# liuzl/rwkv-tts-rs

Measured on AMD Instinct MI355X. Metric: audio samples/sec (16 kHz) for RWKV-TTS 0.4B, batch=32 per GPU, higher is better.
Workload: dtype bf16; 1 GPU; config3: 32 requests/GPU, P=32 prompt, 32 global + 512 semantic tokens, exact sampler, + BiCodec vocoder -> PCM (vocoder of batch s overlapped with LM of batch s+1 on its own stream); global_batch=32, seq_len=577, parallelism=dp1 (request sharding)

## Files before the change

### rwkv-tts-rs_amd/csrc/sampler.hip

```cpp
#include "sampler.h"
#include "exact_math.h"

namespace rwkvtts {

__device__ inline uint32_t rotl32(uint32_t x, int n) { return (x << n) | (x >> (32 - n)); }
#define QR(a, b, c, d)               \
  a += b; d ^= a; d = rotl32(d, 16); \
  c += d; b ^= c; b = rotl32(b, 12); \
  a += b; d ^= a; d = rotl32(d, 8);  \
  c += d; b ^= c; b = rotl32(b, 7);

__device__ uint32_t chacha12_word(const uint32_t* key, uint64_t index) {
  uint32_t in[16] = {0x61707865u, 0x3320646eu, 0x79622d32u, 0x6b206574u};
  for (int i = 0; i < 8; ++i) in[4 + i] = key[i];
  const uint64_t ctr = index >> 4;
  in[12] = (uint32_t)ctr;
  in[13] = (uint32_t)(ctr >> 32);
  in[14] = 0;
  in[15] = 0;
  uint32_t x[16];
  for (int i = 0; i < 16; ++i) x[i] = in[i];
  for (int i = 0; i < 12; i += 2) {
    QR(x[0], x[4], x[8], x[12]);
    QR(x[1], x[5], x[9], x[13]);
// ... 163 lines not shown
}
__device__ inline float prefix64(float s, float v, float* total) {
  float out = 0.0f;
  const int lane = threadIdx.x & 63;
#pragma unroll 8
  for (int i = 0; i < 64; ++i) {
    s += readlane_f(v, i);
    out = lane == i ? s : out;
  }
  *total = s;
  return out;
}

struct SampleSmem {
  float* p;
  uint64_t* keys;
  int* list;
  int* scan;
  double* dscan;
  uint32_t* sub_t;
  int* sub_e;
  int* chunk_e;
  uint32_t* chunk_t;
  int* chunk_ok;
  int* runs;
  uint64_t* etab;
  float* fred;
  int* ired;
  int cap;
};

__device__ inline int wave_sum_i(int v) {
  for (int o = 32; o >= 1; o >>= 1) v += __shfl_xor(v, o);
  return v;
}

template <int NT>
__device__ inline float block_max(float v, float* fred) {
  for (int o = 32; o >= 1; o >>= 1) v = fmaxf(v, __shfl_xor(v, o));
  __syncthreads();
  if ((threadIdx.x & 63) == 0) fred[threadIdx.x >> 6] = v;
  __syncthreads();
  float m = fred[0];
#pragma unroll
  for (int w = 1; w < NT / 64; ++w) m = fmaxf(m, fred[w]);
  return m;
}

template <int N>
__device__ inline int dpp_shr(int v) {
  return __builtin_amdgcn_update_dpp(0, v, 0x110 + N, 0xF, 0xF, false);
}
template <int N>
__device__ inline double dpp_shr(double v) {
  const uint64_t u = __builtin_bit_cast(uint64_t, v);
  const uint32_t lo = (uint32_t)dpp_shr<N>((int)(uint32_t)u), hi = (uint32_t)dpp_shr<N>((int)(uint32_t)(u >> 32));
  return __builtin_bit_cast(double, ((uint64_t)hi << 32) | lo);
}
template <int N>
__device__ inline uint32_t dpp_shr(uint32_t v) {
  return (uint32_t)dpp_shr<N>((int)v);
}
__device__ inline double readlane_d(double v, int l) {
  const uint64_t u = __builtin_bit_cast(uint64_t, v);
  const uint32_t lo = (uint32_t)__builtin_amdgcn_readlane((int)(uint32_t)u, l);
  const uint32_t hi = (uint32_t)__builtin_amdgcn_readlane((int)(uint32_t)(u >> 32), l);
  return __builtin_bit_cast(double, ((uint64_t)hi << 32) | lo);
}
__device__ inline double wave_incl_scan_d(double x) {
  x += dpp_shr<1>(x);
  x += dpp_shr<2>(x);
  x += dpp_shr<4>(x);
  x += dpp_shr<8>(x);
  const double r0 = readlane_d(x, 15), r1 = readlane_d(x, 31), r2 = readlane_d(x, 47);
  const int row = (threadIdx.x & 63) >> 4;
  return x + (row == 0 ? 0.0 : (row == 1 ? r0 : (row == 2 ? r0 + r1 : (r0 + r1) + r2)));
}

__device__ inline uint64_t readlane_u64(uint64_t v, int l) {
  const uint32_t lo = (uint32_t)__builtin_amdgcn_readlane((int)(uint32_t)v, l);
  const uint32_t hi = (uint32_t)__builtin_amdgcn_readlane((int)(uint32_t)(v >> 32), l);
  return ((uint64_t)hi << 32) | lo;
}
template <typename KeyAt>
__device__ inline int wave_rank_gt(uint64_t q, int m, const KeyAt& key_at) {
  const int lane = threadIdx.x & 63;
  int rank = 0;
  for (int j0 = 0; j0 < m; j0 += 64) {
    const uint64_t kl = j0 + lane < m ? key_at(j0 + lane) : 0ull;
#pragma unroll
    for (int j = 0; j < 64; ++j) rank += readlane_u64(kl, j) > q ? 1 : 0;
  }
  return rank;
}
__device__ inline int readlane_t(int v, int l) { return __builtin_amdgcn_readlane(v, l); }
__device__ inline uint32_t readlane_t(uint32_t v, int l) { return (uint32_t)__builtin_amdgcn_readlane((int)v, l); }
__device__ inline double readlane_t(double v, int l) { return readlane_d(v, l); }

template <int NT, typename T>
__device__ inline T block_excl_scan_t(T v, T* scratch, T* tot) {
  const int lane = threadIdx.x & 63, w = threadIdx.x >> 6;
  T x = v;
  x += dpp_shr<1>(x);
  x += dpp_shr<2>(x);
  x += dpp_shr<4>(x);
  x += dpp_shr<8>(x);
  {
    const T r0 = readlane_t(x, 15), r1 = readlane_t(x, 31), r2 = readlane_t(x, 47);
    const int row = lane >> 4;
    const T off = row == 0 ? (T)0 : (row == 1 ? r0 : (row == 2 ? r0 + r1 : (r0 + r1) + r2));
    x += off;
  }
  __syncthreads();
  if (lane == 63) scratch[w] = x;
  __syncthreads();
  T base = 0;
  for (int k = 0; k < w; ++k) base += scratch[k];
  T t = scratch[0];
#pragma unroll
  for (int k = 1; k < NT / 64; ++k) t += scratch[k];
  *tot = t;
  return base + x - v;
}
template <int NT>
__device__ inline int block_excl_scan(int v, int* scratch, int* tot) { return block_excl_scan_t<NT, int>(v, scratch, tot); }

template <int NT>
__device__ int compact_positive_(const float* p, int* list, int* scan, int cap, int n) {
  const int chunk = (n + NT - 1) / NT;
  const int b = min(n, (int)threadIdx.x * chunk), e = min(n, b + chunk);
  int cnt = 0;
  for (int i = b; i < e; ++i) cnt += p[i] > 0.0f;
  int tot;
  int off = block_excl_scan<NT>(cnt, scan, &tot);
  for (int i = b; i < e; ++i)
    if (p[i] > 0.0f) {
      if (off < cap) list[off] = i;
      ++off;
    }
  __syncthreads();
  return tot;
}
template <int NT>
__device__ inline int compact_positive(const SampleSmem& sm, int n) {
  return compact_positive_<NT>(sm.p, sm.list, sm.scan, sm.cap, n);
}

__device__ float wave_sum_positive_(const float* p, const int* list, int cap, int n, int npos) {
  const int lane = threadIdx.x & 63;
  float s = 0.0f;
  if (npos <= cap) {
    for (int q0 = 0; q0 < npos; q0 += 64) {
      const float v = (q0 + lane < npos) ? p[list[q0 + lane]] : 0.0f;
      const int cnt = min(64, npos - q0);
      for (int i = 0; i < cnt; ++i) s += readlane_f(v, i);
    }
  } else {
    for (int q0 = 0; q0 < n; q0 += 64) {
      const float v = (q0 + lane < n) ? p[q0 + lane] : 0.0f;
      const int cnt = min(64, n - q0);
      for (int i = 0; i < cnt; ++i) s += readlane_f(v, i);
    }
  }
  return s;
}
__device__ inline float wave_sum_positive(const SampleSmem& sm, int n, int npos) {
  return wave_sum_positive_(sm.p, sm.list, sm.cap, n, npos);
}

__device__ inline void sum_sim_elem(uint32_t b, int E, uint32_t& T0, uint32_t& T1, int& q0, int& q1, bool& ok) {
  const uint32_t ef = (b >> 23) & 0xFFu;
  uint32_t M = b & 0x7FFFFFu;
  int ex;
  if (ef == 0) ex = -149;
  else { M |= 0x800000u; ex = (int)ef - 150; }
  uint32_t a = 0;
  int cls = 0;
  if (M != 0) {
    const int sh = (E - 23) - ex;
    if (sh <= 0) {
// ... 319 lines not shown
      const uint32_t T1 = (uint32_t)readlane_i((int)(hiw ? b1 : b0), l);
      if (rs < pos) {
        serial(pos, re);
        pos = max(pos, re);
        continue;
      }
      serial(pos, rs);
      s = __builtin_bit_cast(float, __builtin_amdgcn_readfirstlane(__builtin_bit_cast(int, s)));
      const uint32_t sb = __builtin_bit_cast(uint32_t, s);
      const int ef = (int)((sb >> 23) & 0xFFu);
      const uint32_t mm = (sb & 0x7FFFFFu) | 0x800000u;
      const uint32_t T = (mm & 1u) ? T1 : T0;
      if (ef != 0 && ef - 127 == k + kRunEMin && mm + T < 0x1000000u)
        s = __builtin_bit_cast(float, (sb & 0xFF800000u) | ((mm + T) & 0x7FFFFFu));
      else
        serial(rs, re);
      pos = re;
    }
    serial(pos, n);
    if (tid == 0) {
      sm.fred[16] = s;
      if (stamps) {
        stamps[14] = __builtin_amdgcn_s_memtime();
        stamps[15] = sadd;
      }
    }
  } else {
    other();
  }
  __syncthreads();
  STAMP(13);
  return sm.fred[16];
}

template <int NT, typename Other = NoOther>
__device__ __attribute__((always_inline)) float exact_seq_sum(const SampleSmem& sm, int n, uint64_t* stamps = nullptr, const Other& other = Other()) {
  if (n <= kSampleMaxN) return exact_seq_sum_runs<NT>(sm, n, stamps, other);
  return exact_seq_sum_chunks<NT>(sm, n, stamps, other);
}

template <int NT>
__device__ void bitonic_desc(uint64_t* keys, int M) {
  for (int k = 2; k <= M; k <<= 1) {
    for (int j = k >> 1; j > 0; j >>= 1) {
      for (int q = threadIdx.x; q < M; q += NT) {
        const int ixj = q ^ j;
        if (ixj > q) {
          const uint64_t A = keys[q], B = keys[ixj];
          const bool desc = (q & k) == 0;
          if (desc ? (A < B) : (A > B)) { keys[q] = B; keys[ixj] = A; }
        }
      }
      __syncthreads();
    }
  }
}

template <int NT>
__device__ void sort_desc_u32(uint32_t* v, int n) {
  int M = 1;
  while (M < n) M <<= 1;
  for (int k = 2; k <= M; k <<= 1) {
    for (int j = k >> 1; j > 0; j >>= 1) {
      const bool flip = j == (k >> 1);
      for (int t = threadIdx.x; t < (M >> 1); t += NT) {
        const int q = ((t & ~(j - 1)) << 1) | (t & (j - 1));
        const int ixj = flip ? (q ^ (2 * j - 1)) : (q | j);
        if (ixj < n) {
          const uint32_t A = v[q], B = v[ixj];
          if (A < B) { v[q] = B; v[ixj] = A; }
        }
      }
      __syncthreads();
    }
  }
}

__device__ inline uint64_t pkey(float p, int i) {
  return ((uint64_t)__builtin_bit_cast(uint32_t, p) << 32) | (uint64_t)(0xFFFFFFFFu - (uint32_t)i);
}

constexpr int kSampleMaxVals = (kSampleMaxSorted * 8 + 16 * 8 + kSampleMaxSorted * 4) / 4;
constexpr int kFastK = kFastTopK;
constexpr int kFastCap = 1024;
static_assert(kSampleMaxSorted >= 2048 + kFastCap, "fast-path key regions");

__device__ inline bool sample_fast_ok(float sum, float L, int nc, int top_k) {
  if (!(sum > 0.0f) || !(L > 0.0f) || nc < top_k || nc > kFastCap) return false;
  const float P = L / sum;
  return P >= 0x1p-126f && P <= 1.0f;
}

__device__ inline float draw_r(const uint32_t* key, uint64_t draw, bool fixed42) {
  if (!fixed42) return draw_f32(key, draw);
  uint32_t k42[8];
  uint64_t st = 42;
  const uint64_t MUL = 6364136223846793005ull, INC = 11634580456473284103ull;
  for (int i = 0; i < 8; ++i) {
    st = st * MUL + INC;
    const uint32_t xs = (uint32_t)(((st >> 18) ^ st) >> 27);
    const uint32_t rot = (uint32_t)(st >> 59);
    k42[i] = (xs >> rot) | (xs << ((32 - rot) & 31));
  }
  return draw_f32(k42, 0);
}

template <int NT>
__device__ __attribute__((always_inline)) int sample_fast(const SampleSmem& sm, int nc, float sum, float top_p,
                                                          int top_k, float tinv, const uint32_t* key, uint64_t draw,
                                                          bool fixed42, float* dbg, uint64_t* stamps) {
  const int tid = threadIdx.x;
  uint64_t* pk = sm.keys + 2048;
  for (int c = tid; c < nc; c += NT) {
    const uint64_t ce = sm.keys[c];
    pk[c] = pkey(__builtin_bit_cast(float, (uint32_t)(ce >> 32)) / sum, (int)(uint32_t)ce);
  }
  __syncthreads();
  STAMP(4);
  for (int c = tid; c < nc; c += NT) {
    const uint64_t kc = pk[c];
    int rank = 0;
    for (int j = 0; j < nc; ++j) rank += pk[j] > kc ? 1 : 0;
    if (rank < top_k) sm.keys[rank] = kc;
  }
  __syncthreads();
  STAMP(5);
  STAMP(6);
  if (tid < 64) {
    int m = top_k, found = 0, ceq = 0;
    float cutoff = 0.0f;
    if (top_p < 1.0f) {
      float cum = 0.0f;
      for (int q0 = 0; q0 < top_k && !found; q0 += 64) {
        const bool in = q0 + tid < top_k;
        const float pv = in ? __builtin_bit_cast(float, (uint32_t)(sm.keys[q0 + tid] >> 32)) : 0.0f;
        float tot;
        const float pre = prefix64(cum, pv, &tot);
        const uint64_t hit = __ballot(in && pre >= top_p);
        if (hit) {
          found = 1;
          cutoff = readlane_f(pv, __builtin_ctzll(hit));
        }
        cum = tot;
      }
      if (found) {
        m = 0;
        for (int q0 = 0; q0 < top_k; q0 += 64) {
          const bool in = q0 + tid < top_k;
          const float pv = in ? __builtin_bit_cast(float, (uint32_t)(sm.keys[q0 + tid] >> 32)) : 0.0f;
          m += __popcll(__ballot(in && pv >= cutoff));
          ceq += __popcll(__ballot(in && pv == cutoff));
        }
      }
    }
    if (tid == 0) {
      sm.ired[2] = found;
      sm.ired[3] = ceq;
      sm.ired[6] = m;
      sm.fred[17] = cutoff;
    }
  }
  __syncthreads();
  const int m = sm.ired[6];
  for (int t = tid; t < m; t += NT) {
    const uint64_t kt = sm.keys[t];
    const uint32_t lt = (uint32_t)kt;
// ... 71 lines not shown
        for (int q0 = 0; q0 < m && ret < 0; q0 += 64) {
          const bool in = q0 + tid < m;
          const int idx_l = in ? sm.list[q0 + tid] : 0;
          const float v = in ? sm.p[idx_l] : 0.0f;
          float tot;
          const float pre = prefix64(cum, v, &tot);
          const uint64_t hit = __ballot(in && r <= pre);
          const uint64_t posm = __ballot(in && v > 0.0f);
          if (posm) last_pos = readlane_i(idx_l, 63 - __builtin_clzll(posm));
          if (hit) ret = readlane_i(idx_l, __builtin_ctzll(hit));
          cum = tot;
        }
        if (ret < 0) ret = max(last_pos, 0);
      }
      if (tid == 0) {
        sm.ired[5] = ret;
        if (dbg) { dbg[0] = sum; dbg[1] = r; }
      }
    }
    __syncthreads();
    STAMP(9);
    return sm.ired[5];
  }
  if (tid < 64) {
    const int found = sm.ired[2], ceq = sm.ired[3];
    const float cutoff = sm.fred[17];
    bool adj_on = false;
    float adj = 0.0f;
    if (top_p < 1.0f && found && top_p > 0.0f) {
      float s2 = 0.0f;
      for (int q0 = 0; q0 < m; q0 += 64) {
        const float v = q0 + tid < m ? sm.p[sm.list[q0 + tid]] : 0.0f;
        const int cnt = min(64, m - q0);
        for (int i = 0; i < cnt; ++i) s2 += readlane_f(v, i);
      }
      if (s2 < top_p && ceq > 0) {
        adj = (top_p - s2) / (float)ceq;
        adj_on = true;
      }
    }
    const float r = sm.fred[21];
    int ret = -1;
    if (r <= 0.0f) {
      ret = 0;
    } else {
      float cum = 0.0f;
      for (int q0 = 0; q0 < m && ret < 0; q0 += 64) {
        const bool in = q0 + tid < m;
        const int idx_l = in ? sm.list[q0 + tid] : 0;
        float v = in ? sm.p[idx_l] : 0.0f;
        if (adj_on && in && v == cutoff) v = cutoff + adj;
        float tot;
        const float pre = prefix64(cum, v, &tot);
        const uint64_t hit = __ballot(in && r <= pre);
        if (hit) ret = readlane_i(idx_l, __builtin_ctzll(hit));
        cum = tot;
      }
      if (ret < 0) ret = sm.list[m - 1];
    }
    if (tid == 0) {
      sm.ired[5] = ret;
      if (dbg) { dbg[0] = sum; dbg[1] = r; }
    }
  }
  __syncthreads();
  STAMP(9);
  return sm.ired[5];
}

__device__ inline double crude_sum_eps(int n) { return (double)n * 0x1p-23 + 0x1p-36; }

template <int NT>
__device__ __attribute__((always_inline)) int sample_cert(const SampleSmem& sm, int n, int nc, double E, float r, float top_p, int top_k,
                           double eps, uint64_t* stamps = nullptr) {
  const int tid = threadIdx.x;
  STAMP(7);
  uint64_t* srt = sm.keys + 2048;
  uint64_t* idx_o = sm.keys + 3072;
  static_assert(kSampleMaxSorted >= 3072 + kFastK, "certified-path key regions");
  auto qkey = [&](int j) {
    const uint64_t kj = sm.keys[j];
    return (kj & 0xFFFFFFFF00000000ull) | (uint64_t)(0xFFFFFFFFu - (uint32_t)kj);
  };
  for (int c0 = 0; c0 < nc; c0 += NT) {
    if (c0 + (tid & ~63) >= nc) break;
    const int c = c0 + tid;
    const uint64_t qc = c < nc ? qkey(c) : ~0ull;
    const int rank = wave_rank_gt(qc, nc, qkey);
    if (c < nc) srt[rank] = qc;
  }
  __syncthreads();
  STAMP(8);
  for (int t0 = 0; t0 < top_k; t0 += NT) {
    if (t0 + (tid & ~63) >= top_k) break;
    const int t = t0 + tid;
    const uint64_t kt = t < top_k ? srt[t] : 0ull;
    const uint32_t it = 0xFFFFFFFFu - (uint32_t)kt;
    auto nkey = [&](int j) { return (uint64_t)(uint32_t)srt[j]; };
    const int ri = wave_rank_gt((uint64_t)(uint32_t)kt, top_k, nkey);
    if (t < top_k) idx_o[ri] = (kt & 0xFFFFFFFF00000000ull) | it;
  }
  __syncthreads();
  STAMP(9);
  int ret = -1;
  if (tid < 64) {
    const double s_lo = E * (1.0 - eps), s_hi = E * (1.0 + eps);
    const double u = 0x1p-24, ua = 0x1p-23;
    bool ok = E > 0.0 && s_lo > 0.0 && E < 3.0e38;
    const float ek = __builtin_bit_cast(float, (uint32_t)(srt[top_k - 1] >> 32));
    if (ok && nc > top_k) {
      const float eb = __builtin_bit_cast(float, (uint32_t)(srt[top_k] >> 32));
      ok = (double)ek >= (double)eb * (1.0 + 0x1p-22);
    }
    ok = ok && (double)ek / s_hi >= 0x1p-120;
    double tot_hi = 0.0;
    for (int q0 = 0; q0 < top_k; q0 += 64) {
      const double e = q0 + tid < top_k ? (double)__builtin_bit_cast(float, (uint32_t)(idx_o[q0 + tid] >> 32)) : 0.0;
      tot_hi += readlane_d(wave_incl_scan_d(e), 63);
    }
    tot_hi = tot_hi / s_lo * (1.0 + u) * (1.0 + (double)top_k * ua);
    if (top_p < 1.0f) ok = ok && tot_hi < (double)top_p;
    STAMP(12);
    if (ok) {
      if (r <= 0.0f) {
        ret = 0;
      } else {
        double plo = 0.0, phi = 0.0, hi_prev = 0.0;
        bool amb = false;
        for (int q0 = 0; q0 < top_k && ret < 0 && !amb; q0 += 64) {
          const bool in = q0 + tid < top_k;
          const uint64_t kv = in ? idx_o[q0 + tid] : 0ull;
          const double e = in ? (double)__builtin_bit_cast(float, (uint32_t)(kv >> 32)) : 0.0;
          const double a = wave_incl_scan_d(e / s_hi * (1.0 - u)), b = wave_incl_scan_d(e / s_lo * (1.0 + u));
          const int j = q0 + tid;
          const double lo = (plo + a) * (1.0 - (double)(j + 1) * ua);
          const double hi = (phi + b) * (1.0 + (double)(j + 1) * ua);
          const uint64_t le = __ballot(in && (double)r <= lo);
          const uint64_t hm = __ballot(in && (double)r <= hi);
          if (le) {
            const int f = __builtin_ctzll(le);
            const int fh = __builtin_ctzll(hm);
            if (fh == f && (f > 0 || hi_prev < (double)r)) ret = __builtin_amdgcn_readlane((int)(uint32_t)kv, f);
            else amb = true;
          } else if (hm) {
            amb = true;
          }
          plo = readlane_d(plo + a, 63);
          phi = readlane_d(phi + b, 63);
          hi_prev = phi * (1.0 + (double)min(q0 + 64, top_k) * ua);
        }
        if (ret < 0 && !amb) ret = (int)(uint32_t)idx_o[top_k - 1];
        if (amb) ret = -1;
      }
    }
    if (tid == 0) sm.ired[7] = ret;
  }
  STAMP(13);
  __syncthreads();
  return sm.ired[7];
}

template <int NT, bool kValSort = true>
__device__ __attribute__((always_inline)) int sample_block(const SampleSmem& sm, int n, float temperature, float top_p,
                            int top_k, const uint32_t* key, uint64_t draw, bool fixed42,
                            float* dbg, int* status, uint64_t* stamps = nullptr, bool cert = true,
                            bool prepped = false) {
  const int tid = threadIdx.x;
  *status = 0;
  if (n == 0) return 0;
  if (!prepped) STAMP(1);
  if (!prepped) {
  float mx = -__builtin_inff();
  if (tid < 32) sm.etab[tid] = exp2_tab(tid);
  for (int i = tid; i < n; i += NT) mx = fmaxf(mx, sm.p[i]);
  mx = block_max<NT>(mx, sm.fred);
  {
    const uint64_t* et = sm.etab;
    auto tab = [et](int i) { return et[i]; };
    int i = tid;
    for (; i + 3 * NT < n; i += 4 * NT) {
      const float x0 = sm.p[i], x1 = sm.p[i + NT], x2 = sm.p[i + 2 * NT], x3 = sm.p[i + 3 * NT];
      sm.p[i] = glibc_expf_t(x0 - mx, tab);
      sm.p[i + NT] = glibc_expf_t(x1 - mx, tab);
      sm.p[i + 2 * NT] = glibc_expf_t(x2 - mx, tab);
      sm.p[i + 3 * NT] = glibc_expf_t(x3 - mx, tab);
    }
    for (; i < n; i += NT) sm.p[i] = glibc_expf_t(sm.p[i] - mx, tab);
  }
  }
  static_assert(NT <= 512, "fred[8 + wave] per candidate wave");
  const bool temp_on = temperature != 1.0f && temperature > 0.0f;
  const bool want_fast = top_k > 0 && top_k < n && top_k <= kFastK;
  if (tid == 0 && !prepped) {
    sm.ired[30] = 0;
    sm.ired[31] = 0;
    sm.fred[20] = 0.0f;
  }
  __syncthreads();
  STAMP(2);
  auto collect = [&]() {
    if (!want_fast) return;
    constexpr int NC = NT - 64, NWC = NT / 64 - 1;
    const int ct = tid - 64, lane = tid & 63;
    float lm = -1.0f;
    for (int i = ct; i < n; i += NC) lm = fmaxf(lm, sm.p[i]);
    const int kw = (top_k + NWC - 1) / NWC;
    int gt = 0, ge = 0;
#pragma unroll 16
    for (int j = 0; j < 64; ++j) {
      const float o = readlane_f(lm, j);
      gt += o > lm ? 1 : 0;
      ge += o >= lm ? 1 : 0;
    }
    const uint64_t selm = __ballot(gt < kw && kw <= ge);
    const float vw = readlane_f(lm, __builtin_ctzll(selm));
    if (lane == 0) {
      sm.fred[8 + (tid >> 6)] = vw;
      __hip_atomic_fetch_add(&sm.ired[30], 1, __ATOMIC_RELEASE, __HIP_MEMORY_SCOPE_WORKGROUP);
    }
    while (__hip_atomic_load(&sm.ired[30], __ATOMIC_ACQUIRE, __HIP_MEMORY_SCOPE_WORKGROUP) < NWC)
      __builtin_amdgcn_s_sleep(1);
    float L = sm.fred[9];
#pragma unroll
    for (int w = 2; w < NT / 64; ++w) L = fminf(L, sm.fred[8 + w]);
    if (!(L > 0.0f)) return;
    if (tid == 64) sm.fred[20] = L;
    const float T = L * (1.0f - 0x1p-19f);
    for (int i0 = 0; i0 < n; i0 += NC) {
      const int i = i0 + ct;
      const float v = i < n ? sm.p[i] : 0.0f;
      const bool c = i < n && v >= T;
      const uint64_t bm = __ballot(c);
      if (bm) {
        int base = 0;
        if (lane == 0) base = atomicAdd(&sm.ired[31], __popcll(bm));
        base = __builtin_amdgcn_readfirstlane(base);
        const int off = base + __popcll(bm & ((1ull << lane) - 1ull));
        if (c && off < kFastCap) sm.keys[off] = ((uint64_t)__builtin_bit_cast(uint32_t, v) << 32) | (uint32_t)i;
      }
    }
  };
  auto other = [&]() {
    collect();
    if (tid == NT - 64) sm.fred[21] = draw_r(key, draw, fixed42);
  };
  bool other_done = prepped;
  if (prepped) {
    const int nc = sm.ired[31];
    const float L = sm.fred[20];
    if (want_fast && !temp_on && !dbg && cert && n <= kSampleMaxN && L > 0.0f && nc >= top_k && nc <= kFastCap) {
      const int ret = sample_cert<NT>(sm, n, nc, sm.dscan[12], sm.fred[21], top_p, top_k, sm.dscan[13], stamps);
      STAMP(11);
      if (ret >= 0) return ret;
    }
  } else if (want_fast && !temp_on && !dbg && cert && n <= kSampleMaxN) {
    if (tid < 64) {
      double e = 0.0;
      for (int i = tid; i < n; i += 64) e += (double)sm.p[i];
      for (int o = 32; o >= 1; o >>= 1) e += __shfl_xor(e, o);
      if (tid == 0) sm.dscan[12] = e;
    } else {
      other();
    }
    __syncthreads();
    STAMP(10);
    other_done = true;
    const int nc = sm.ired[31];
    const float L = sm.fred[20];
    if (L > 0.0f && nc >= top_k && nc <= kFastCap) {
      const int ret = sample_cert<NT>(sm, n, nc, sm.dscan[12], sm.fred[21], top_p, top_k, crude_sum_eps(n));
      STAMP(11);
      if (ret >= 0) return ret;
    }
  }
  auto other_once = [&]() {
    if (!other_done) other();
  };
  const float sum = exact_seq_sum<NT>(sm, n, stamps, other_once);
  STAMP(3);
  if (want_fast) {
    const int nc = sm.ired[31];
    const float L = sm.fred[20];
    if (sample_fast_ok(sum, L, nc, top_k))
      return sample_fast<NT>(sm, nc, sum, top_p, top_k, temp_on ? 1.0f / temperature : 0.0f, key, draw, fixed42, dbg, stamps);
  }
  if (sum > 0.0f)
    for (int i = tid; i < n; i += NT) sm.p[i] = sm.p[i] / sum;
  __syncthreads();
  STAMP(4);
  int n_sorted = -1;
  if (top_k > 0 && top_k < n) {
    bool done = false;
    if (top_k <= 64 * (NT / 64)) {
      const int chunk = (n + NT - 1) / NT;
      const int b = min(n, tid * chunk), e = min(n, b + chunk);
      float lm = -1.0f;
      for (int i = b; i < e; ++i) lm = fmaxf(lm, sm.p[i]);
      const int lane = tid & 63;
      const int kw = (top_k + NT / 64 - 1) / (NT / 64);
      int gt = 0, ge = 0;
#pragma unroll 16
      for (int j = 0; j < 64; ++j) {
        const float o = readlane_f(lm, j);
        gt += o > lm ? 1 : 0;
        ge += o >= lm ? 1 : 0;
      }
      const uint64_t selm = __ballot(gt < kw && kw <= ge);
      const float vw = readlane_f(lm, __builtin_ctzll(selm));
      if (lane == 0) sm.fred[tid >> 6] = vw;
      __syncthreads();
      float Lm = sm.fred[0];
#pragma unroll
      for (int w = 1; w < NT / 64; ++w) Lm = fminf(Lm, sm.fred[w]);
      const float L = fmaxf(Lm, 0.0f);
      int cnt = 0;
      for (int i = b; i < e; ++i) cnt += sm.p[i] >= L;
      int tot;
      int off = block_excl_scan<NT>(cnt, sm.scan, &tot);
      if (tot <= sm.cap) {
        for (int i = b; i < e; ++i)
          if (sm.p[i] >= L) sm.keys[off++] = pkey(sm.p[i], i);
        if (tot <= NT) {
          __syncthreads();
          const uint64_t kq = tid < tot ? sm.keys[tid] : 0ull;
          int rank = 0;
          if (tid < tot)
            for (int j = 0; j < tot; ++j) rank += sm.keys[j] > kq ? 1 : 0;
          __syncthreads();
          if (tid < tot) sm.keys[rank] = kq;
          __syncthreads();
        } else {
          int M = 1;
          while (M < tot) M <<= 1;
          for (int q = tot + tid; q < M; q += NT) sm.keys[q] = 0ull;
          __syncthreads();
// ... 253 lines not shown
  char* g = a.scratch + (size_t)row * a.scratch_stride;
  SampleSmem sm = carve<NT>(smem, 0, false);
  sm.p = (float*)g;
  sm.keys = (uint64_t*)(g + (size_t)((a.n + 3) & ~3) * 4);
  sm.list = (int*)((char*)sm.keys + (size_t)wide_keys_len(a.n) * 8);
  sm.cap = a.n;
  uint64_t* stamps = a.stamps ? a.stamps + row * 16 : nullptr;
  STAMP(0);
  const float* lg = a.logits + (int64_t)row * a.ld;
  for (int i = threadIdx.x; i < a.n; i += NT) sm.p[i] = lg[i];
  __syncthreads();
  if (threadIdx.x == 0 && a.forbid >= 0 && a.forbid < a.n) sm.p[a.forbid] = -__builtin_inff();
  __syncthreads();
  int status;
  const int id = sample_block<NT>(sm, a.n, a.temperature, a.top_p, a.top_k,
                              a.keys ? a.keys + row * 8 : nullptr, a.draws ? a.draws[row] : 0,
                              a.keys == nullptr, a.dbg ? a.dbg + row * 2 : nullptr, &status, stamps);
  if (threadIdx.x == 0) a.out[row] = status ? status : id;
}

void launch_sample_rows(const SampleRowArgs& a, int rows, hipStream_t st) {
  if (a.n > kSampleMaxN) {
    const size_t lds = smem_bytes<kSampleThreads>(0) - kSampleMaxSorted * 12;
    RT_LAUNCH(k_sample_rows_wide, dim3(rows), dim3(kSampleThreads), lds, st, a);
    return;
  }
  RT_LAUNCH(k_sample_rows, dim3(rows), dim3(kSampleThreads), smem_bytes<kSampleThreads>(a.n), st, a);
}

__device__ inline float load_logit(const AdvanceArgs& a, const float* lg, int i) {
  float v = lg[i];
  for (int p = 1; p < a.n_part; ++p) v += lg[p * a.part_stride + i];
  return v;
}

template <int NT>
__device__ inline void load_logits_row(const AdvanceArgs& a, const float* lg, float* p, int n) {
  int i = threadIdx.x;
  for (; i + 3 * NT < n; i += 4 * NT) {
    float v[4];
#pragma unroll
    for (int u = 0; u < 4; ++u) v[u] = lg[i + u * NT];
    for (int q = 1; q < a.n_part; ++q) {
      float w[4];
#pragma unroll
      for (int u = 0; u < 4; ++u) w[u] = lg[q * a.part_stride + i + u * NT];
#pragma unroll
      for (int u = 0; u < 4; ++u) v[u] += w[u];
    }
#pragma unroll
    for (int u = 0; u < 4; ++u) p[i + u * NT] = v[u];
  }
  for (; i < n; i += NT) p[i] = load_logit(a, lg, i);
}

template <int NT, int PT>
__device__ __attribute__((always_inline)) void advance_load_row(const AdvanceArgs& a, const float* lg, float* v) {
  const int last = a.ld - 1, tid = threadIdx.x;
#pragma unroll
  for (int k = 0; k < PT; ++k) v[k] = lg[min(tid + k * NT, last)];
  if (a.n_part == 2) {
    float w[PT];
#pragma unroll
    for (int k = 0; k < PT; ++k) w[k] = lg[a.part_stride + min(tid + k * NT, last)];
#pragma unroll
    for (int k = 0; k < PT; ++k) v[k] += w[k];
  } else if (a.n_part == 4) {
    float w[3][PT];
#pragma unroll
    for (int q = 0; q < 3; ++q)
#pragma unroll
      for (int k = 0; k < PT; ++k) w[q][k] = lg[(q + 1) * a.part_stride + min(tid + k * NT, last)];
#pragma unroll
    for (int q = 0; q < 3; ++q)
#pragma unroll
      for (int k = 0; k < PT; ++k) v[k] += w[q][k];
  } else {
    for (int q = 1; q < a.n_part; ++q)
#pragma unroll
      for (int k = 0; k < PT; ++k) v[k] += lg[q * a.part_stride + min(tid + k * NT, last)];
  }
}

template <int NT, int N, int PT>
__device__ __attribute__((always_inline)) void advance_prep(const float* raw, const SampleSmem& sm, bool mask_eos,
                                                            int top_k, const uint32_t* key, uint64_t draw,
                                                            uint32_t* blk, uint64_t* blk_id, uint64_t* stamps) {
  constexpr int NW = NT / 64, n = N;
  static_assert(PT * NT >= N, "row registers");
  const int masked = mask_eos ? N - 1 : -1;
  const int tid = threadIdx.x, lane = tid & 63, wave = tid >> 6;
  float v[PT];
#pragma unroll
  for (int k = 0; k < PT; ++k) v[k] = raw[k];
  if (tid == NT - 64) sm.fred[21] = draw_cached(key, draw, blk, blk_id);
  if (tid < 32) sm.etab[tid] = exp2_tab(tid);
  if (tid == 0) sm.ired[31] = 0;
  float mx = -__builtin_inff();
#pragma unroll
  for (int k = 0; k < PT; ++k) {
    const int i = tid + k * NT;
    if (i == masked) v[k] = -__builtin_inff();
    if (i < n) mx = fmaxf(mx, v[k]);
  }
  STAMP(1);
  mx = block_max<NT>(mx, sm.fred);
  STAMP(3);
  const uint64_t* et = sm.etab;
  auto tab = [et](int j) { return et[j]; };
  double es = 0.0;
  float lm = -1.0f;
#pragma unroll
  for (int k = 0; k < PT; ++k) {
    const int i = tid + k * NT;
    if (i < n) {
      const float e = glibc_expf_t(v[k] - mx, tab);
      v[k] = e;
      sm.p[i] = e;
      es += (double)e;
      lm = fmaxf(lm, e);
    }
  }
  STAMP(4);
  es = readlane_d(wave_incl_scan_d(es), 63);
  const bool want = top_k > 0 && top_k < n && top_k <= kFastK;
  if (want) {
    const int kw = (top_k + NW - 1) / NW;
    int gt = 0, ge = 0;
#pragma unroll 16
    for (int j = 0; j < 64; ++j) {
      const float o = readlane_f(lm, j);
      gt += o > lm ? 1 : 0;
      ge += o >= lm ? 1 : 0;
    }
    const uint64_t selm = __ballot(gt < kw && kw <= ge);
    const float vw = readlane_f(lm, __builtin_ctzll(selm));
    if (lane == 0) sm.fred[8 + wave] = vw;
  }
  if (lane == 0) sm.dscan[wave] = es;
  STAMP(5);
  __syncthreads();
  STAMP(6);
  float L = 0.0f;
  if (want) {
    L = sm.fred[8];
#pragma unroll
    for (int w = 1; w < NW; ++w) L = fminf(L, sm.fred[8 + w]);
  }
  if (L > 0.0f) {
    const float T = L * (1.0f - 0x1p-19f);
    uint64_t bms[PT];
    int tot = 0;
#pragma unroll
    for (int k = 0; k < PT; ++k) {
      const int i = tid + k * NT;
      bms[k] = __ballot(i < n && v[k] >= T);
      tot += __popcll(bms[k]);
    }
    if (tot) {
      int base = 0;
      if (lane == 0) base = atomicAdd(&sm.ired[31], tot);
      base = __builtin_amdgcn_readfirstlane(base);
#pragma unroll
      for (int k = 0; k < PT; ++k) {
        const int i = tid + k * NT;
        const int off = base + __popcll(bms[k] & ((1ull << lane) - 1ull));
        if (((bms[k] >> lane) & 1ull) && off < kFastCap)
          sm.keys[off] = ((uint64_t)__builtin_bit_cast(uint32_t, v[k]) << 32) | (uint32_t)i;
        base += __popcll(bms[k]);
      }
    }
  }
  STAMP(14);
  double E = sm.dscan[0];
#pragma unroll
  for (int w = 1; w < NW; ++w) E += sm.dscan[w];
  {
    double* dbuf = (double*)sm.list;
    constexpr int C = (N + NT - 1) / NT, G = NT / 64;
    const int b = min(n, tid * C), e = min(n, b + C);
    double ts = 0.0;
    for (int i = b; i < e; ++i) ts += (double)sm.p[i];
    dbuf[tid] = ts;
    __syncthreads();
    if (tid < 64) {
      double g[G], acc = 0.0;
#pragma unroll
      for (int q = 0; q < G; ++q) {
        g[q] = dbuf[lane * G + q];
        acc += g[q];
      }
      double run = wave_incl_scan_d(acc) - acc;
#pragma unroll
      for (int q = 0; q < G; ++q) {
        dbuf[NT + lane * G + q] = run;
        run += g[q];
      }
    }
    __syncthreads();
    const double up = 1.0 + crude_sum_eps(n) + 0x1p-30;
    double P = dbuf[NT + tid], bp = 0.0;
    for (int i = b; i < e; ++i) {
      P += (double)sm.p[i];
      if (i > 0) {
        const int k = max((int)((__builtin_bit_cast(uint64_t, P * up) >> 52) & 0x7FF) - 1023, -126);
        bp += __builtin_bit_cast(double, (uint64_t)(k - 24 + 1023) << 52);
      }
    }
    dbuf[tid] = bp;
    __syncthreads();
    if (tid < 64) {
      double acc = 0.0;
#pragma unroll
      for (int q = 0; q < G; ++q) acc += dbuf[lane * G + q];
      const double B = readlane_d(wave_incl_scan_d(acc), 63);
      if (tid == 0) sm.dscan[13] = B / E * (1.0 + 0x1p-30) + 0x1p-36;
    }
  }
  if (tid == 0) {
    sm.dscan[12] = E;
    sm.fred[20] = L;
  }
  __syncthreads();
  STAMP(10);
}

template <int NT, int PT>
__device__ __attribute__((always_inline)) void advance_penalise(float* raw, uint16_t* cnt, int n_sem, float rep, float freq,
                                                                float pres) {
  const int tid = threadIdx.x;
  if (n_sem == 0) {
#pragma unroll
    for (int k = 0; k < PT; ++k) {
      const int i = tid + k * NT;
      if (i < kPenCounts) cnt[i] = 0;
    }
    return;
  }
  uint32_t cn[PT];
#pragma unroll
  for (int k = 0; k < PT; ++k) {
    const int i = tid + k * NT;
    cn[k] = i < kPenCounts ? cnt[i] : 0u;
  }
#pragma unroll
  for (int k = 0; k < PT; ++k) {
    if (cn[k] == 0u) continue;
    float x = raw[k];
    if (rep != 1.0f) {
      for (uint32_t r = 0; r < cn[k]; ++r) {
        const float y = x > 0.0f ? __fdiv_rn(x, rep) : __fmul_rn(x, rep);
        if (__builtin_bit_cast(uint32_t, y) == __builtin_bit_cast(uint32_t, x)) break;
        x = y;
      }
    }
    if (freq != 0.0f) x = __fsub_rn(x, __fmul_rn(freq, (float)cn[k]));
    if (pres != 0.0f) x = __fsub_rn(x, pres);
    raw[k] = x;
  }
}

template <bool kParams>
__device__ __attribute__((always_inline)) void advance_body(const AdvanceArgs& a, char* smem) {
  constexpr int NT = kSampleThreads;
  const int row = blockIdx.x;
  uint64_t* stamps = a.stamps ? a.stamps + row * 16 : nullptr;
  STAMP(0);
  constexpr int NS = RWKVTTS_EOS_TOKEN + 1, PT = (NS + NT - 1) / NT;
  const float* lg = a.logits + (int64_t)row * a.ld;
  float raw[PT];
  advance_load_row<NT, PT>(a, lg, raw);
  const int slot = a.row_slot[row];
  SlotCtrl* c = a.ctrl + slot;
  const int phase = c->phase;
  __syncthreads();
  if (phase == kPhDone) return;
  if (phase == kPhGFeed) {
    if (threadIdx.x == 0) {
      c->next_token = RWKVTTS_TAG_1;
      c->phase = c->sem_limit > 0 ? kPhSemantic : kPhDone;
    }
    return;
  }
  const bool glob = phase == kPhGlobal;
  const SampleSmem sm = carve<NT>(smem, NS);
  const bool eos_masked = !glob && (c->fixed || (c->mode == 1 && c->n_sem < c->hard_min));
  const int n = glob ? 4096 : NS, top_k = glob ? c->top_k_g : c->top_k_s;
  const float temp = !kParams ? 1.0f : (glob ? c->temp_g : c->temp_s);
  const float top_p = !kParams ? 0.95f : (glob ? c->top_p_g : c->top_p_s);
  const uint32_t* key = glob ? c->gkey : c->skey;
  const uint64_t draw = glob ? c->gdraw : c->sdraw;
  bool pen = false;
  uint16_t* pen_cnt = nullptr;
  if constexpr (kParams) {
    const float rep = a.pen[slot].repetition, freq = a.pen[slot].frequency, pres = a.pen[slot].presence;
    pen = !glob && (rep != 1.0f || freq != 0.0f || pres != 0.0f);
    if (pen) {
      pen_cnt = a.pen_counts + (int64_t)slot * kPenCounts;
      advance_penalise<NT, PT>(raw, pen_cnt, c->n_sem, rep, freq, pres);
    }
  }
  int id = 0, status;
  uint64_t used = 1;
  bool stop = false, masked = eos_masked;
  for (int attempt = 0; attempt < 2; ++attempt) {
    if (glob) advance_prep<NT, 4096, PT>(raw, sm, false, top_k, key, draw + attempt, c->gblk, &c->gblk_id, stamps);
    else advance_prep<NT, NS, PT>(raw, sm, masked, top_k, key, draw + attempt, c->sblk, &c->sblk_id, stamps);
    id = sample_block<NT, kParams>(sm, n, temp, top_p, top_k, key, draw + attempt, false, nullptr, &status, stamps,
                          a.cert != 0, true);
    used = attempt + 1;
    if (glob || id != RWKVTTS_EOS_TOKEN) break;
    if (c->mode == 0) {
      stop = true;
      break;
    }
    const int wl = c->win_len;
    const int non_eos = __builtin_popcount((uint32_t)c->win_bits & ((1u << wl) - 1u));
    const float ratio = wl > 0 ? (float)non_eos / (float)wl : 0.0f;
    if (wl >= 12 && ratio >= 0.7f) {
      stop = true;
      break;
    }
    masked = true;
    __syncthreads();
  }
  STAMP(15);
  if (glob) {
    if (threadIdx.x == 0) {
      c->gdraw += 1;
      c->global_out[c->n_global++] = id;
      c->next_token = id + RWKVTTS_GLOBAL_TOKEN_OFFSET;
      if (c->n_global == RWKVTTS_N_GLOBAL) c->phase = kPhGFeed;
    }
    return;
  }
  if (threadIdx.x == 0) {
    c->sdraw += used;
    if (stop) {
      c->phase = kPhDone;
    } else {
      if (c->mode == 1) {
        c->win_bits = ((c->win_bits << 1) | (id != RWKVTTS_EOS_TOKEN ? 1 : 0)) & 0xFFF;
        if (c->win_len < 12) c->win_len++;
      }
      a.sem_out[(int64_t)slot * RWKVTTS_SEMANTIC_LIMIT + c->n_sem] = id;
      if constexpr (kParams) {
        if (pen) {
          const int W = a.pen[slot].window, ns = c->n_sem;
          if ((uint32_t)id < (uint32_t)kPenCounts) pen_cnt[id] += 1;
          if (W > 0 && ns >= W) {
            const int old = a.sem_out[(int64_t)slot * RWKVTTS_SEMANTIC_LIMIT + ns - W];
            if ((uint32_t)old < (uint32_t)kPenCounts) pen_cnt[old] -= 1;
          }
        }
      }
      c->n_sem++;
      c->next_token = id;
      if (c->n_sem >= c->sem_limit) c->phase = kPhDone;
    }
  }
}

__global__ __launch_bounds__(kSampleThreads, 2) void k_advance(AdvanceArgs a) {
  extern __shared__ __attribute__((aligned(16))) char smem[];
  tl_begin(a.tl);
  advance_body<false>(a, smem);
  tl_end(a.tl);
}
__global__ __launch_bounds__(kSampleThreads, 2) void k_advance_params(AdvanceArgs a) {
  extern __shared__ __attribute__((aligned(16))) char smem[];
  tl_begin(a.tl);
  advance_body<true>(a, smem);
  tl_end(a.tl);
}

int launch_advance(const AdvanceArgs& a0, hipStream_t st, int cert) {
  AdvanceArgs a = a0;
  a.cert = cert;
  const size_t lds = smem_bytes<kSampleThreads>(RWKVTTS_EOS_TOKEN + 1);
  if (a.params) RT_LAUNCH(k_advance_params, dim3(a.n_rows), dim3(kSampleThreads), lds, st, a);
  else RT_LAUNCH(k_advance, dim3(a.n_rows), dim3(kSampleThreads), lds, st, a);
  return a.n_rows;
}

}
```

Measured before the change: 11.42 million samples/s.

## Restructure advance sampler: block-split ranking, bitwise threshold, fused prefix scan, 512 threads

Replaces the per-wave rank sort in the certified sampling path with a block-wide ranking that splits the comparison range across idle waves and then sums partial ranks. The per-wave top-k threshold now uses a bitwise radix search with ballots instead of a 64-lane readlane loop. The mass and error-bound prefix scans are rewritten as register-resident chunked wave scans with fewer barriers, and E/eps are returned in registers. The advance kernel is pinned to 512 threads, control fields are cached in locals, and optional stamp-gated statistics atomics are added. This trades extra LDS partial buffers and more complex indexing for less serial per-wave work and fewer barriers in the per-token sampler.

```diff
diff --git a/rwkv-tts-rs_amd/csrc/sampler.hip b/rwkv-tts-rs_amd/csrc/sampler.hip
--- a/rwkv-tts-rs_amd/csrc/sampler.hip
+++ b/rwkv-tts-rs_amd/csrc/sampler.hip
@@ -269,20 +269,39 @@
   const uint32_t hi = (uint32_t)__builtin_amdgcn_readlane((int)(uint32_t)(v >> 32), l);
   return ((uint64_t)hi << 32) | lo;
 }
-template <typename KeyAt>
-__device__ inline int wave_rank_gt(uint64_t q, int m, const KeyAt& key_at) {
-  const int lane = threadIdx.x & 63;
-  int rank = 0;
-  for (int j0 = 0; j0 < m; j0 += 64) {
-    const uint64_t kl = j0 + lane < m ? key_at(j0 + lane) : 0ull;
-#pragma unroll
-    for (int j = 0; j < 64; ++j) rank += readlane_u64(kl, j) > q ? 1 : 0;
-  }
-  return rank;
-}
 __device__ inline int readlane_t(int v, int l) { return __builtin_amdgcn_readlane(v, l); }
 __device__ inline uint32_t readlane_t(uint32_t v, int l) { return (uint32_t)__builtin_amdgcn_readlane((int)v, l); }
 __device__ inline double readlane_t(double v, int l) { return readlane_d(v, l); }
+__device__ inline uint64_t readlane_t(uint64_t v, int l) { return readlane_u64(v, l); }
+template <int NT, typename K, typename KeyAt, typename Emit>
+__device__ inline void block_rank_gt(int m_any, int* part, const KeyAt& key_at, const Emit& emit) {
+  constexpr int NW = NT / 64;
+  const int m = __builtin_amdgcn_readfirstlane(m_any);
+  const int tid = threadIdx.x, lane = tid & 63, wave = __builtin_amdgcn_readfirstlane(tid >> 6);
+  const int QB = (m + 63) >> 6, LS = QB >= NW ? 0 : 31 - __builtin_clz(NW / QB), SP = 1 << LS;
+  const int SL = (((m + SP - 1) >> LS) + 15) & ~15, stride = QB * 64;
+  for (int t = wave; t < QB * SP; t += NW) {
+    const int qb = t >> LS, seg = t & (SP - 1), c = qb * 64 + lane;
+    const K q = c < m ? key_at(c) : ~(K)0;
+    const int jb = min(m, seg * SL), je = min(m, jb + SL);
+    int rank = 0;
+    for (int j0 = jb; j0 < je; j0 += 64) {
+      const K kl = j0 + lane < je ? key_at(j0 + lane) : (K)0;
+      const int cnt = min(64, je - j0);
+      for (int g = 0; g < cnt; g += 16) {
+#pragma unroll
+        for (int j = 0; j < 16; ++j) rank += readlane_t(kl, g + j) > q ? 1 : 0;
+      }
+    }
+    part[seg * stride + c] = rank;
+  }
+  __syncthreads();
+  for (int c = tid; c < m; c += NT) {
+    int rank = 0;
+    for (int sg = 0; sg < SP; ++sg) rank += part[sg * stride + c];
+    emit(c, rank);
+  }
+}
 
 template <int NT, typename T>
 __device__ inline T block_excl_scan_t(T v, T* scratch, T* tot) {
@@ -768,6 +787,7 @@
 
 constexpr int kSampleMaxVals = (kSampleMaxSorted * 8 + 16 * 8 + kSampleMaxSorted * 4) / 4;
 constexpr int kFastK = kFastTopK;
+constexpr int kCertOutcome = 40;
 constexpr int kFastCap = 1024;
 static_assert(kSampleMaxSorted >= 2048 + kFastCap, "fast-path key regions");
 
@@ -1005,24 +1025,16 @@
     const uint64_t kj = sm.keys[j];
     return (kj & 0xFFFFFFFF00000000ull) | (uint64_t)(0xFFFFFFFFu - (uint32_t)kj);
   };
-  for (int c0 = 0; c0 < nc; c0 += NT) {
-    if (c0 + (tid & ~63) >= nc) break;
-    const int c = c0 + tid;
-    const uint64_t qc = c < nc ? qkey(c) : ~0ull;
-    const int rank = wave_rank_gt(qc, nc, qkey);
-    if (c < nc) srt[rank] = qc;
-  }
+  int* part = sm.list + 64;
+  static_assert(kSampleMaxSorted >= 64 + kFastCap && kFastCap >= NT, "partial-rank buffer");
+  block_rank_gt<NT, uint64_t>(nc, part, qkey, [&](int c, int rank) { srt[rank] = qkey(c); });
   __syncthreads();
   STAMP(8);
-  for (int t0 = 0; t0 < top_k; t0 += NT) {
-    if (t0 + (tid & ~63) >= top_k) break;
-    const int t = t0 + tid;
-    const uint64_t kt = t < top_k ? srt[t] : 0ull;
-    const uint32_t it = 0xFFFFFFFFu - (uint32_t)kt;
-    auto nkey = [&](int j) { return (uint64_t)(uint32_t)srt[j]; };
-    const int ri = wave_rank_gt((uint64_t)(uint32_t)kt, top_k, nkey);
-    if (t < top_k) idx_o[ri] = (kt & 0xFFFFFFFF00000000ull) | it;
-  }
+  auto nkey = [&](int j) { return (uint32_t)srt[j]; };
+  block_rank_gt<NT, uint32_t>(top_k, part, nkey, [&](int t, int ri) {
+    const uint64_t kt = srt[t];
+    idx_o[ri] = (kt & 0xFFFFFFFF00000000ull) | (0xFFFFFFFFu - (uint32_t)kt);
+  });
   __syncthreads();
   STAMP(9);
   int ret = -1;
@@ -1087,7 +1099,7 @@
 __device__ __attribute__((always_inline)) int sample_block(const SampleSmem& sm, int n, float temperature, float top_p,
                             int top_k, const uint32_t* key, uint64_t draw, bool fixed42,
                             float* dbg, int* status, uint64_t* stamps = nullptr, bool cert = true,
-                            bool prepped = false) {
+                            bool prepped = false, double prep_E = 0.0, double prep_eps = 0.0) {
   const int tid = threadIdx.x;
   *status = 0;
   if (n == 0) return 0;
@@ -1172,8 +1184,9 @@
     const int nc = sm.ired[31];
     const float L = sm.fred[20];
     if (want_fast && !temp_on && !dbg && cert && n <= kSampleMaxN && L > 0.0f && nc >= top_k && nc <= kFastCap) {
-      const int ret = sample_cert<NT>(sm, n, nc, sm.dscan[12], sm.fred[21], top_p, top_k, sm.dscan[13], stamps);
+      const int ret = sample_cert<NT>(sm, n, nc, prep_E, sm.fred[21], top_p, top_k, prep_eps, stamps);
       STAMP(11);
+      if (stamps && tid == 0) sm.ired[kCertOutcome] = ret >= 0 ? 1 : 2;
       if (ret >= 0) return ret;
     }
   } else if (want_fast && !temp_on && !dbg && cert && n <= kSampleMaxN) {
@@ -1593,8 +1606,12 @@
   }
 }
 
+struct AdvancePrep {
+  double E;
+  double eps;
+};
 template <int NT, int N, int PT>
-__device__ __attribute__((always_inline)) void advance_prep(const float* raw, const SampleSmem& sm, bool mask_eos,
+__device__ __attribute__((always_inline)) AdvancePrep advance_prep(const float* raw, const SampleSmem& sm, bool mask_eos,
                                                             int top_k, const uint32_t* key, uint64_t draw,
                                                             uint32_t* blk, uint64_t* blk_id, uint64_t* stamps) {
   constexpr int NW = NT / 64, n = N;
@@ -1606,7 +1623,10 @@
   for (int k = 0; k < PT; ++k) v[k] = raw[k];
   if (tid == NT - 64) sm.fred[21] = draw_cached(key, draw, blk, blk_id);
   if (tid < 32) sm.etab[tid] = exp2_tab(tid);
-  if (tid == 0) sm.ired[31] = 0;
+  if (tid == 0) {
+    sm.ired[31] = 0;
+    sm.ired[kCertOutcome] = 0;
+  }
   float mx = -__builtin_inff();
 #pragma unroll
   for (int k = 0; k < PT; ++k) {
@@ -1619,7 +1639,6 @@
   STAMP(3);
   const uint64_t* et = sm.etab;
   auto tab = [et](int j) { return et[j]; };
-  double es = 0.0;
   float lm = -1.0f;
 #pragma unroll
   for (int k = 0; k < PT; ++k) {
@@ -1628,27 +1647,23 @@
       const float e = glibc_expf_t(v[k] - mx, tab);
       v[k] = e;
       sm.p[i] = e;
-      es += (double)e;
       lm = fmaxf(lm, e);
     }
   }
   STAMP(4);
-  es = readlane_d(wave_incl_scan_d(es), 63);
   const bool want = top_k > 0 && top_k < n && top_k <= kFastK;
   if (want) {
+    static_assert(N >= NT, "every thread owns an element: lm >= 0");
     const int kw = (top_k + NW - 1) / NW;
-    int gt = 0, ge = 0;
-#pragma unroll 16
-    for (int j = 0; j < 64; ++j) {
-      const float o = readlane_f(lm, j);
-      gt += o > lm ? 1 : 0;
-      ge += o >= lm ? 1 : 0;
-    }
-    const uint64_t selm = __ballot(gt < kw && kw <= ge);
-    const float vw = readlane_f(lm, __builtin_ctzll(selm));
-    if (lane == 0) sm.fred[8 + wave] = vw;
-  }
-  if (lane == 0) sm.dscan[wave] = es;
+    const uint32_t lb = __builtin_bit_cast(uint32_t, lm);
+    uint32_t t = 0u;
+#pragma unroll
+    for (int bit = 30; bit >= 0; --bit) {
+      const uint32_t cand = t | (1u << bit);
+      if (__popcll(__ballot(lb >= cand)) >= kw) t = cand;
+    }
+    if (lane == 0) sm.fred[8 + wave] = __builtin_bit_cast(float, t);
+  }
   STAMP(5);
   __syncthreads();
   STAMP(6);
@@ -1683,57 +1698,54 @@
     }
   }
   STAMP(14);
-  double E = sm.dscan[0];
-#pragma unroll
-  for (int w = 1; w < NW; ++w) E += sm.dscan[w];
+  if (tid == 0) sm.fred[20] = L;
+  AdvancePrep out;
   {
-    double* dbuf = (double*)sm.list;
-    constexpr int C = (N + NT - 1) / NT, G = NT / 64;
-    const int b = min(n, tid * C), e = min(n, b + C);
+    double* wtot = (double*)sm.list;
+    constexpr int C = ((N + NT - 1) / NT) | 1;
+    static_assert(C * NT >= N && 2 * NW * 8 <= kSampleMaxSorted * 4, "chunk layout");
+    const int b = min(n, tid * C);
+    float c[C];
+#pragma unroll
+    for (int j = 0; j < C; ++j) c[j] = b + j < n ? sm.p[b + j] : 0.0f;
     double ts = 0.0;
-    for (int i = b; i < e; ++i) ts += (double)sm.p[i];
-    dbuf[tid] = ts;
+#pragma unroll
+    for (int j = 0; j < C; ++j) ts += (double)c[j];
+    const double incl = wave_incl_scan_d(ts);
+    double P = __shfl_up(incl, 1);
+    if (lane == 0) P = 0.0;
+    if (lane == 63) wtot[wave] = incl;
     __syncthreads();
-    if (tid < 64) {
-      double g[G], acc = 0.0;
-#pragma unroll
-      for (int q = 0; q < G; ++q) {
-        g[q] = dbuf[lane * G + q];
-        acc += g[q];
-      }
-      double run = wave_incl_scan_d(acc) - acc;
-#pragma unroll
-      for (int q = 0; q < G; ++q) {
-        dbuf[NT + lane * G + q] = run;
-        run += g[q];
-      }
-    }
-    __syncthreads();
+    double E = 0.0, base = 0.0;
+#pragma unroll
+    for (int w = 0; w < NW; ++w) {
+      const double t = wtot[w];
+      base += w < wave ? t : 0.0;
+      E += t;
+    }
+    P += base;
     const double up = 1.0 + crude_sum_eps(n) + 0x1p-30;
-    double P = dbuf[NT + tid], bp = 0.0;
-    for (int i = b; i < e; ++i) {
-      P += (double)sm.p[i];
-      if (i > 0) {
+    double bp = 0.0;
+#pragma unroll
+    for (int j = 0; j < C; ++j) {
+      P += (double)c[j];
+      const int i = b + j;
+      if (i > 0 && i < n) {
         const int k = max((int)((__builtin_bit_cast(uint64_t, P * up) >> 52) & 0x7FF) - 1023, -126);
         bp += __builtin_bit_cast(double, (uint64_t)(k - 24 + 1023) << 52);
       }
     }
-    dbuf[tid] = bp;
+    bp = wave_incl_scan_d(bp);
+    if (lane == 63) wtot[NW + wave] = bp;
     __syncthreads();
-    if (tid < 64) {
-      double acc = 0.0;
-#pragma unroll
-      for (int q = 0; q < G; ++q) acc += dbuf[lane * G + q];
-      const double B = readlane_d(wave_incl_scan_d(acc), 63);
-      if (tid == 0) sm.dscan[13] = B / E * (1.0 + 0x1p-30) + 0x1p-36;
-    }
-  }
-  if (tid == 0) {
-    sm.dscan[12] = E;
-    sm.fred[20] = L;
-  }
-  __syncthreads();
+    double B = 0.0;
+#pragma unroll
+    for (int w = 0; w < NW; ++w) B += wtot[NW + w];
+    out.E = E;
+    out.eps = B / E * (1.0 + 0x1p-30) + 0x1p-36;
+  }
   STAMP(10);
+  return out;
 }
 
 template <int NT, int PT>
@@ -1771,9 +1783,11 @@
   }
 }
 
+constexpr int kAdvanceThreads = 512;
+
 template <bool kParams>
 __device__ __attribute__((always_inline)) void advance_body(const AdvanceArgs& a, char* smem) {
-  constexpr int NT = kSampleThreads;
+  constexpr int NT = kAdvanceThreads;
   const int row = blockIdx.x;
   uint64_t* stamps = a.stamps ? a.stamps + row * 16 : nullptr;
   STAMP(0);
@@ -1784,6 +1798,9 @@
   const int slot = a.row_slot[row];
   SlotCtrl* c = a.ctrl + slot;
   const int phase = c->phase;
+  const int c_mode = c->mode, c_fixed = c->fixed, c_n_sem = c->n_sem, c_hard_min = c->hard_min;
+  const int c_top_k_g = c->top_k_g, c_top_k_s = c->top_k_s;
+  const uint64_t c_gdraw = c->gdraw, c_sdraw = c->sdraw;
   __syncthreads();
   if (phase == kPhDone) return;
   if (phase == kPhGFeed) {
@@ -1795,12 +1812,12 @@
   }
   const bool glob = phase == kPhGlobal;
   const SampleSmem sm = carve<NT>(smem, NS);
-  const bool eos_masked = !glob && (c->fixed || (c->mode == 1 && c->n_sem < c->hard_min));
-  const int n = glob ? 4096 : NS, top_k = glob ? c->top_k_g : c->top_k_s;
+  const bool eos_masked = !glob && (c_fixed || (c_mode == 1 && c_n_sem < c_hard_min));
+  const int n = glob ? 4096 : NS, top_k = glob ? c_top_k_g : c_top_k_s;
   const float temp = !kParams ? 1.0f : (glob ? c->temp_g : c->temp_s);
   const float top_p = !kParams ? 0.95f : (glob ? c->top_p_g : c->top_p_s);
   const uint32_t* key = glob ? c->gkey : c->skey;
-  const uint64_t draw = glob ? c->gdraw : c->sdraw;
+  const uint64_t draw = glob ? c_gdraw : c_sdraw;
   bool pen = false;
   uint16_t* pen_cnt = nullptr;
   if constexpr (kParams) {
@@ -1808,17 +1825,18 @@
     pen = !glob && (rep != 1.0f || freq != 0.0f || pres != 0.0f);
     if (pen) {
       pen_cnt = a.pen_counts + (int64_t)slot * kPenCounts;
-      advance_penalise<NT, PT>(raw, pen_cnt, c->n_sem, rep, freq, pres);
+      advance_penalise<NT, PT>(raw, pen_cnt, c_n_sem, rep, freq, pres);
     }
   }
   int id = 0, status;
   uint64_t used = 1;
   bool stop = false, masked = eos_masked;
   for (int attempt = 0; attempt < 2; ++attempt) {
-    if (glob) advance_prep<NT, 4096, PT>(raw, sm, false, top_k, key, draw + attempt, c->gblk, &c->gblk_id, stamps);
-    else advance_prep<NT, NS, PT>(raw, sm, masked, top_k, key, draw + attempt, c->sblk, &c->sblk_id, stamps);
+    const AdvancePrep pr =
+        glob ? advance_prep<NT, 4096, PT>(raw, sm, false, top_k, key, draw + attempt, c->gblk, &c->gblk_id, stamps)
+             : advance_prep<NT, NS, PT>(raw, sm, masked, top_k, key, draw + attempt, c->sblk, &c->sblk_id, stamps);
     id = sample_block<NT, kParams>(sm, n, temp, top_p, top_k, key, draw + attempt, false, nullptr, &status, stamps,
-                          a.cert != 0, true);
+                          a.cert != 0, true, pr.E, pr.eps);
     used = attempt + 1;
     if (glob || id != RWKVTTS_EOS_TOKEN) break;
     if (c->mode == 0) {
@@ -1836,6 +1854,17 @@
     __syncthreads();
   }
   STAMP(15);
+  if (stamps && threadIdx.x == 0) {
+    unsigned long long* acc = (unsigned long long*)a.stamps + 255 * 16;
+    const unsigned long long dt = stamps[15] - stamps[0];
+    atomicAdd(acc + 0, dt);
+    atomicAdd(acc + 1, 1ull);
+    atomicMax(acc + 2, dt);
+    const int co = sm.ired[kCertOutcome];
+    if (co == 0) atomicAdd(acc + 3, 1ull);
+    if (co == 2) atomicAdd(acc + 4, 1ull);
+    atomicAdd(acc + 5, (unsigned long long)sm.ired[31]);
+  }
   if (glob) {
     if (threadIdx.x == 0) {
       c->gdraw += 1;
@@ -1872,13 +1901,13 @@
   }
 }
 
-__global__ __launch_bounds__(kSampleThreads, 2) void k_advance(AdvanceArgs a) {
+__global__ __launch_bounds__(kAdvanceThreads, 2) void k_advance(AdvanceArgs a) {
   extern __shared__ __attribute__((aligned(16))) char smem[];
   tl_begin(a.tl);
   advance_body<false>(a, smem);
   tl_end(a.tl);
 }
-__global__ __launch_bounds__(kSampleThreads, 2) void k_advance_params(AdvanceArgs a) {
+__global__ __launch_bounds__(kAdvanceThreads, 2) void k_advance_params(AdvanceArgs a) {
   extern __shared__ __attribute__((aligned(16))) char smem[];
   tl_begin(a.tl);
   advance_body<true>(a, smem);
@@ -1888,9 +1917,9 @@
 int launch_advance(const AdvanceArgs& a0, hipStream_t st, int cert) {
   AdvanceArgs a = a0;
   a.cert = cert;
-  const size_t lds = smem_bytes<kSampleThreads>(RWKVTTS_EOS_TOKEN + 1);
-  if (a.params) RT_LAUNCH(k_advance_params, dim3(a.n_rows), dim3(kSampleThreads), lds, st, a);
-  else RT_LAUNCH(k_advance, dim3(a.n_rows), dim3(kSampleThreads), lds, st, a);
+  const size_t lds = smem_bytes<kAdvanceThreads>(RWKVTTS_EOS_TOKEN + 1);
+  if (a.params) RT_LAUNCH(k_advance_params, dim3(a.n_rows), dim3(kAdvanceThreads), lds, st, a);
+  else RT_LAUNCH(k_advance, dim3(a.n_rows), dim3(kAdvanceThreads), lds, st, a);
   return a.n_rows;
 }
 
```

Result: no change. 11.42 million samples/s (-0.0%).
